# nreHieW/Eagle

Hardware: AMD Instinct MI355X
Metric: frames/sec end-to-end (detect+keypoint+homography) @1280x720 (higher is better)
Workload: dtype f32 (split: hi/lo binary16 pairs, 3 x fp16 MFMA per product, fp32 accumulate); detector (1.4 % of the FLOP): f32, exact v_mfma_f32_16x16x4_f32 chains

## Files before the change

eagle_amd/csrc/conv.hip:

```cpp
#include <algorithm>
#include <cmath>
#include <cstdlib>
#include <mutex>

#include "common.h"
#include "dmath.h"
#include "conv_internal.h"

namespace eagle {

static int f16_ps(int kc) { const int g = kc / 8; return kc * 2 + ((g % 2 == 0) ? 16 : 0); }
static int f16_ni(int ks, int kc) { return (ks * ks * (kc / 8) + 3) / 4; }

enum FormKind { GENERIC, WSTAT, ADIRECT };
enum StrideForm { S1, S2D, S2T };
enum WeightImage { W_F32, W_F16, W_F16_S2D, W_SPLIT, W_SPLIT_AD, W_SPLIT_S2D, W_SPLIT_M32 };
struct Form {
    int prec, variant, kind;
    int pw;
    int sform, rows, cols;
    int kc, nt, halo_bufs;
    int wimage;
    int grid_cap;
    ConvKernelGetter get;
};
static constexpr Form gen(int prec, int variant, int pw, int wimage, int kind = GENERIC) { return {prec, variant, kind, pw, S1, 0, 0, 0, 0, 0, wimage, 0, nullptr}; }
static constexpr Form ad(int prec, int variant, int sform, int rows, int cols, int nt, int halo_bufs, int wimage, ConvKernelGetter get, int grid_cap = 0)
{
    return {prec, variant, ADIRECT, 0, sform, rows, cols, prec == EAGLE_PREC_F16 ? 32 : 16, nt, halo_bufs, wimage, grid_cap, get};
}
static constexpr int F16 = EAGLE_PREC_F16, F32 = EAGLE_PREC_F32, F32S = EAGLE_PREC_F32S;
static constexpr Form g_forms[] = {
    gen(F32, 0, 4, W_F32), gen(F32, 3, 2, W_F32), gen(F32, 4, 1, W_F32),
    gen(F16, 0, 4, W_F16), gen(F16, 2, 4, W_F16), gen(F16, 3, 2, W_F16), gen(F16, 4, 1, W_F16), gen(F16, 6, 4, W_F16, WSTAT), gen(F16, 7, 2, W_F16, WSTAT),
    ad(F16, 8, S1, 4, 32, 12, 2, W_F16, conv_ad_kernel_s1_bn192), ad(F16, 9, S1, 8, 32, 6, 2, W_F16, conv_ad_kernel_s1_bn96),
    ad(F16, 10, S2D, 4, 32, 12, 2, W_F16_S2D, conv_ad_kernel_s2_bn192), ad(F16, 11, S2D, 8, 32, 6, 2, W_F16_S2D, conv_ad_kernel_s2_bn96),
    gen(F32S, 0, 4, W_SPLIT), gen(F32S, 3, 2, W_SPLIT), gen(F32S, 18, 6, W_SPLIT),
    ad(F32S, 8, S1, 4, 32, 12, 2, W_SPLIT_AD, conv_ad_split_kernel_bn192), ad(F32S, 9, S1, 8, 32, 6, 2, W_SPLIT_AD, conv_ad_split_kernel_bn96),
    ad(F32S, 10, S2D, 4, 32, 12, 2, W_SPLIT_S2D, conv_ad_split_kernel_s2_bn192), ad(F32S, 11, S2D, 8, 32, 6, 2, W_SPLIT_S2D, conv_ad_split_kernel_s2_bn96),
    ad(F32S, 12, S1, 8, 32, 3, 2, W_SPLIT_AD, conv_ad_split_kernel48), ad(F32S, 13, S1, 16, 32, 3, 1, W_SPLIT_AD, conv_ad_split_kernel48sb),
    ad(F32S, 19, S1, 16, 32, 3, 2, W_SPLIT_AD, conv_ad_split_kernel48ring, 256),
    ad(F32S, 14, S2T, 4, 32, 12, 1, W_SPLIT_AD, conv_ad_split_kernel_s2t_bn192), ad(F32S, 15, S2T, 4, 32, 6, 1, W_SPLIT_AD, conv_ad_split_kernel_s2t_bn96),
    ad(F32S, 21, S1, 4, 32, 12, 2, W_SPLIT_M32, conv_ad_split32_kernel_bn192), ad(F32S, 22, S1, 8, 32, 6, 2, W_SPLIT_M32, conv_ad_split32_kernel_bn96),
    ad(F32S, 23, S1, 2, 64, 12, 2, W_SPLIT_M32, conv_ad_split32_kernel_w64_bn192), ad(F32S, 24, S1, 4, 64, 6, 2, W_SPLIT_M32, conv_ad_split32_kernel_w64_bn96)};

static const Form* find_form(int precision, int variant)
{
    for (const Form& f : g_forms)
        if (f.prec == precision && f.variant == variant) return &f;
    return nullptr;
}
static const Form& form_of(int precision, const ConvConfig& c)
{
    const Form* f = find_form(precision, c.variant);
    if (!f) fail(EAGLE_E_NOKERNEL, "no conv kernel form: prec=%d variant=%d", precision, c.variant);
    return *f;
}
static int kind_of(int precision, const ConvConfig& c) { const Form* f = find_form(precision, c.variant); return f ? f->kind : -1; }

static size_t lds_bytes(int precision, const ConvConfig& c)
{
    const Form& f = form_of(precision, c);
    if (f.kind == ADIRECT) {
        int hpix, rec, strips;
        if (precision == EAGLE_PREC_F16) { hpix = f.sform == S2D ? (f.rows + 1) * 33 : (f.rows + 2) * 34; rec = 96; strips = 4 * 32 * 112; }
        else if (f.wimage == W_SPLIT_M32) { hpix = (f.rows + 2) * (f.cols + 2); rec = 80; strips = 4 * 32 * 128; }
        else { hpix = f.sform == S2T ? (2 * f.rows + 1) * 66 : (f.rows + 2) * 34; rec = 96; strips = 4 * 16 * 208; }
        const int slabs = ((hpix * rec + 1023) / 1024 + 3) / 4 * 4;
        return (size_t)f.halo_bufs * slabs * 1024 + strips;
    }
    const int th = 4 * f.pw / c.wx, tw = 16 * c.wx;
    const int hw = (tw - 1) * c.stride + c.ks, hh = (th - 1) * c.stride + c.ks;
    const int bn = c.nt * 16;
    if (precision == EAGLE_PREC_F16) {
        const size_t operands = (size_t)f16_ni(c.ks, c.kc) * 4 * bn * 16 + (size_t)hh * hw * f16_ps(c.kc);
        const size_t strips = (size_t)4 * f.pw * 16 * (bn * 2 + 16);
        return f.kind == WSTAT ? operands + strips + 16 : std::max(operands + 16, strips);
    }
    if (precision == EAGLE_PREC_F32S) {
        const size_t operands = (size_t)f16_ni(c.ks, c.kc) * 2 * 4 * bn * 16 + (size_t)hh * hw * f16_ps(2 * c.kc);
        const size_t strips = (size_t)4 * f.pw * 16 * (bn * 4 + 16);
        return std::max(operands + 16, strips);
    }
    return (size_t)c.ks * c.ks * (c.kc / 4) * 4 * bn * 4 + (size_t)hh * hw * (c.kc + 1) * 4;
}

size_t conv_lds_bytes(int precision, const ConvConfig& c) { return lds_bytes(precision, c); }
void conv_tile_shape(int precision, const ConvConfig& c, int* th, int* tw)
{
    const Form& f = form_of(precision, c);
    *th = f.kind == ADIRECT ? f.rows : 4 * f.pw / c.wx; *tw = f.kind == ADIRECT ? f.cols : 16 * c.wx;
}

int conv_tiles_per_frame(int precision, const ConvConfig& c, int ho, int wo)
{
    int th, tw;
    conv_tile_shape(precision, c, &th, &tw);
    return ((wo + tw - 1) / tw) * ((ho + th - 1) / th);
}

static const Inst* generic_inst(int precision, const ConvConfig& c)
{
    for (auto part : {conv_inst_part0, conv_inst_part1, conv_inst_part2, conv_inst_part3, conv_inst_split0, conv_inst_split1, conv_inst_split2}) {
        int n = 0;
        const Inst* t = part(&n);
        for (int k = 0; k < n; ++k)
            if (t[k].prec == precision && t[k].ks == c.ks && t[k].s == c.stride && t[k].kc == c.kc && t[k].nt == c.nt && t[k].variant == c.variant) return &t[k];
    }
    return nullptr;
}
bool conv_supported(int precision, const ConvConfig& c)
{
    const Form* f = find_form(precision, c.variant);
    if (f && f->kind == ADIRECT) return c.ks == 3 && c.stride == (f->sform == S1 ? 1 : 2) && c.kc == f->kc && c.nt == f->nt;
    return f && generic_inst(precision, c);
}

struct Tuned { int ks, s, cin, cout, wo, kc, nt, wx, variant; };
static const Tuned g_tuned[] = {
#include "conv_tuned.inc"
    {0, 0, 0, 0, 0, 0, 0, 0, 0}};
static const Tuned g_tuned_f32[] = {
#include "conv_tuned_f32.inc"
    {0, 0, 0, 0, 0, 0, 0, 0, 0}};
static const Tuned g_tuned_split[] = {
#include "conv_tuned_split.inc"
    {0, 0, 0, 0, 0, 0, 0, 0, 0}};
static bool tuned_match(const Tuned& t, const ConvConfig& c, int wo, ConvConfig* q)
{
    if (t.ks != c.ks || t.s != c.stride || t.cin != c.cin || t.cout != c.cout_pad || t.wo != wo) return false;
    *q = c; q->kc = t.kc; q->nt = t.nt; q->wx = t.wx; q->variant = t.variant;
    return true;
}

static bool env_force(const char* name, int* a, int* b, int* c) { const char* f = getenv(name); return f && sscanf(f, "%d,%d,%d", a, b, c) == 3; }
static bool env_off(const char* name) { const char* e = getenv(name); return e && atoi(e) == 0; }

static const int g_nts[] = {6, 4, 3, 2, 1};
static ConvConfig with_ad(ConvConfig c, int kc, int v192, int v96)
{
    c.kc = kc;
    if (c.cout_pad % 192 == 0) { c.nt = 12; c.variant = v192; } else { c.nt = 6; c.variant = v96; }
    return c;
}

static ConvConfig choose_f32(ConvConfig c, int wo)
{
    ConvConfig q = c; q.kc = (c.cin < 16) ? 4 : 16;
    if (env_force("EAGLE_F32_FORCE", &q.nt, &q.wx, &q.variant) && (q.wx == 1 || q.wx == 2) && q.nt >= 1 && c.cout_pad % (16 * q.nt) == 0 &&
        conv_supported(EAGLE_PREC_F32, q) && lds_bytes(EAGLE_PREC_F32, q) <= 160 * 1024)
        return q;
    for (const Tuned& t : g_tuned_f32)
        if (tuned_match(t, c, wo, &q) && conv_supported(EAGLE_PREC_F32, q)) return q;
    c.nt = 1;
    for (int nt : g_nts)
        if (c.cout_pad % (16 * nt) == 0) { c.nt = nt; break; }
    c.kc = (c.cin < 16) ? 4 : 16;
    if (c.stride == 2 && c.ks == 3) {
        q = c; q.variant = 3;
        if (conv_supported(EAGLE_PREC_F32, q)) return q;
    }
    return c;
}

static ConvConfig choose_split(ConvConfig c, int wo, bool plain_epilogue)
{
    const int prec = EAGLE_PREC_F32S, cin = c.cin, cout = c.cout_pad;
    ConvConfig q = c;
    if (env_force("EAGLE_CONV_FORCE", &q.kc, &q.nt, &q.variant) && cin % q.kc == 0 && cout % (16 * q.nt) == 0 && conv_supported(prec, q)) {
        if (form_of(prec, q).pw == 6) q.wx = 3;
        if (lds_bytes(prec, q) <= 160 * 1024) return q;
    }
    if (plain_epilogue && c.ks == 3 && c.stride == 2 && cin % 48 == 0 && cout % 96 == 0) return with_ad(c, 16, 14, 15);
    if (!env_off("EAGLE_CONV_M32") && plain_epilogue && c.ks == 3 && c.stride == 1 && cin % 16 == 0 && cout % 96 == 0) return with_ad(c, 16, 21, wo > 32 ? 24 : 22);
    for (const Tuned& t : g_tuned_split)
        if (tuned_match(t, c, wo, &q)) {
            const Form* f = find_form(prec, q.variant);
            if (kind_of(prec, q) == ADIRECT && !(plain_epilogue && cin % (f->sform == S2D ? 16 : 48) == 0)) continue;
            if (conv_supported(prec, q) && lds_bytes(prec, q) <= 160 * 1024) return q;
        }
    if (plain_epilogue && c.ks == 3 && c.stride == 1 && cin % 48 == 0 && cout % 96 == 0) return with_ad(c, 16, 8, 9);
    static const int skcs[] = {32, 16, 8};
    long best = -1;
    c.nt = 1; c.kc = 8; c.variant = 0;
    for (int variant : {0, 3})
        for (int nt : g_nts) {
            if (cout % (16 * nt)) continue;
            for (int kc : skcs) {
                if (cin % kc) continue;
                ConvConfig t = c; t.nt = nt; t.kc = kc; t.variant = variant;
                if (!conv_supported(prec, t)) continue;
                if (lds_bytes(prec, t) > 80 * 1024) continue;
                const int pw = form_of(prec, t).pw;
                if (nt * pw > 12) continue;
                const long score = (long)nt * pw * 1000 + kc * 10 + (variant == 0 ? 1 : 0);
                if (score > best) { best = score; c.nt = nt; c.kc = kc; c.variant = variant; }
            }
        }
    return c;
}

static ConvConfig choose_f16(ConvConfig c, int wo, bool plain_epilogue, bool plain_one)
{
    const int prec = EAGLE_PREC_F16, cin = c.cin, cout = c.cout_pad;
    ConvConfig q = c;
    if (env_force("EAGLE_CONV_FORCE", &q.kc, &q.nt, &q.variant) && cin % q.kc == 0 && cout % (16 * q.nt) == 0 && conv_supported(prec, q) &&
        lds_bytes(prec, q) <= 160 * 1024 && (kind_of(prec, q) == WSTAT ? plain_one : kind_of(prec, q) == ADIRECT ? plain_epilogue : true))
        return q;
    if (plain_epilogue && c.ks == 3 && c.stride == 1 && cin % 32 == 0 && cout % 96 == 0) return with_ad(c, 32, 8, 9);
    if (plain_epilogue && c.ks == 3 && c.stride == 2 && cin % 8 == 0 && cin >= 32 && cout % 96 == 0) return with_ad(c, 32, 10, 11);
    for (const Tuned& t : g_tuned)
        if (tuned_match(t, c, wo, &q)) {
            if (kind_of(prec, q) == WSTAT && !plain_one) continue;
            if (conv_supported(prec, q) && lds_bytes(prec, q) <= 160 * 1024) return q;
        }
    static const int kcs[] = {64, 48, 32, 16, 8};
    long best = -1;
    c.nt = 1; c.kc = 8;
    for (int nt : g_nts) {
        if (cout % (16 * nt)) continue;
        for (int kc : kcs) {
            if (cin % kc) continue;
            ConvConfig t = c; t.nt = nt; t.kc = kc;
            if (!conv_supported(prec, t)) continue;
            if (lds_bytes(prec, t) > 80 * 1024) continue;
            const long score = (long)kc * nt * 1000 + kc;
            if (score > best) { best = score; c.nt = nt; c.kc = kc; }
        }
    }
    return c;
}

ConvConfig conv_choose(int precision, int ks, int stride, int cin_pad, int cout_pad, int wo, bool plain_epilogue, bool second_residual)
{
    ConvConfig c;
    c.ks = ks; c.stride = stride; c.cin = cin_pad; c.cout_pad = cout_pad;
    c.wx = (wo > 16) ? 2 : 1;
    if (precision == EAGLE_PREC_F32) return choose_f32(c, wo);
    if (precision == EAGLE_PREC_F32S) return choose_split(c, wo, plain_epilogue);
    return choose_f16(c, wo, plain_epilogue, plain_epilogue && !second_residual);
}

size_t conv_weight_elems(int precision, const ConvConfig& c)
{
    const int bn = c.nt * 16, nblk = c.cout_pad / bn, nch = c.cin / c.kc;
    switch (form_of(precision, c).wimage) {
    case W_F16_S2D: return (size_t)nblk * (4 * c.cin / 32) * 16 * bn * 8;
    case W_F16: return (size_t)nblk * nch * f16_ni(c.ks, c.kc) * 4 * bn * 8;
    case W_SPLIT_S2D: return (size_t)nblk * (4 * c.cin / 16) * 6 * 4 * bn * 8;
    case W_SPLIT_M32: return (size_t)nblk * (c.cin / 16) * 18 * (bn / 32) * 512;
    case W_SPLIT_AD: return (size_t)nblk * (c.cin / 16) * 14 * 4 * bn * 8;
    case W_SPLIT: return (size_t)nblk * nch * f16_ni(c.ks, c.kc) * 2 * 4 * bn * 8;
    default: return (size_t)nblk * nch * c.ks * c.ks * (c.kc / 4) * 4 * bn;
    }
}

void conv_tile_weights(int precision, const ConvConfig& c, const float* w, int cin_real, int cout_real, void* dst, float* descale)
{
    const int bn = c.nt * 16, nblk = c.cout_pad / bn, nch = c.cin / c.kc, taps = c.ks * c.ks, wimage = form_of(precision, c).wimage;
    auto W = [&](int tap, int ci, int co) -> float {
        return (ci < cin_real && co < cout_real) ? w[((size_t)tap * cin_real + ci) * cout_real + co] : 0.0f;
    };
    if (descale) *descale = 1.0f;
    if (precision == EAGLE_PREC_F32S) {
        float amax = 0.f;
        for (size_t k = 0; k < (size_t)taps * cin_real * cout_real; ++k) amax = std::max(amax, std::fabs(w[k]));
        int e = 0;
        if (amax > 0.f) (void)std::frexp(amax, &e);
        const int sw = 15 - e;
        const float scale = std::ldexp(1.0f, sw);
        if (descale) *descale = std::ldexp(1.0f, -(sw + 4));
        _Float16* d = (_Float16*)dst;
        if (wimage == W_SPLIT_S2D) {
            const int per_phase = c.cin / 16;
            for (int b = 0; b < nblk; ++b)
                for (int ch = 0; ch < 4 * per_phase; ++ch)
                    for (int k = 0; k < 6; ++k)
                        for (int qq = 0; qq < 4; ++qq)
                            for (int nn = 0; nn < bn; ++nn)
                                for (int j = 0; j < 8; ++j) {
                                    const int ph = ch / per_phase, c0 = (ch - ph * per_phase) * 16, ry = ph >> 1, rx = ph & 1;
                                    const int tp = k < 4 ? k : 2 * (k - 4) + (qq >> 1), tyy = tp >> 1, txx = tp & 1;
                                    const int ky = tyy == 0 ? (ry == 1 ? 0 : -1) : (ry == 0 ? 1 : 2), kx = txx == 0 ? (rx == 1 ? 0 : -1) : (rx == 0 ? 1 : 2);
                                    float v = 0.f;
                                    if (ky >= 0 && kx >= 0) v = W(ky * 3 + kx, c0 + (qq & 1) * 8 + j, b * bn + nn) * scale;
                                    const _Float16 hi = (_Float16)v;
                                    *d++ = k < 4 ? hi : (_Float16)(v - (float)hi);
                                }
            return;
        }
        if (wimage == W_SPLIT_M32) {
            for (int b = 0; b < nblk; ++b)
                for (int ch = 0; ch < c.cin / 16; ++ch)
                    for (int tap = 0; tap < 9; ++tap)
                        for (int part = 0; part < 2; ++part)
                            for (int mb = 0; mb < bn / 32; ++mb)
                                for (int l = 0; l < 64; ++l)
                                    for (int j = 0; j < 8; ++j) {
                                        const float v = W(tap, ch * 16 + (l >> 5) * 8 + j, b * bn + mb * 32 + (l & 31)) * scale;
                                        const _Float16 hi = (_Float16)v;
                                        *d++ = part == 0 ? hi : (_Float16)(v - (float)hi);
                                    }
            return;
        }
        if (wimage == W_SPLIT_AD) {
            for (int b = 0; b < nblk; ++b)
                for (int ch = 0; ch < c.cin / 16; ++ch)
                    for (int k = 0; k < 14; ++k)
                        for (int qq = 0; qq < 4; ++qq)
                            for (int nn = 0; nn < bn; ++nn)
                                for (int j = 0; j < 8; ++j) {
                                    const int tap = k < 9 ? k : 2 * (k - 9) + (qq >> 1);
                                    float v = 0.f;
                                    if (tap < 9) v = W(tap, ch * 16 + (qq & 1) * 8 + j, b * bn + nn) * scale;
                                    const _Float16 hi = (_Float16)v;
                                    *d++ = k < 9 ? hi : (_Float16)(v - (float)hi);
                                }
            return;
        }
        const int G = c.kc / 8, NGR = taps * G, NI = f16_ni(c.ks, c.kc);
        for (int b = 0; b < nblk; ++b)
            for (int ch = 0; ch < nch; ++ch)
                for (int i = 0; i < NI; ++i)
                    for (int part = 0; part < 2; ++part)
                        for (int qq = 0; qq < 4; ++qq)
                            for (int nn = 0; nn < bn; ++nn)
                                for (int j = 0; j < 8; ++j) {
                                    const int g = 4 * i + qq;
                                    float v = 0.f;
                                    if (g < NGR) { const int tap = g / G, cg = g % G; v = W(tap, ch * c.kc + cg * 8 + j, b * bn + nn) * scale; }
                                    const _Float16 hi = (_Float16)v;
                                    *d++ = part == 0 ? hi : (_Float16)(v - (float)hi);
                                }
        return;
    }
    if (wimage == W_F16_S2D) {
        _Float16* d = (_Float16*)dst;
        const int nch2 = 4 * c.cin / 32;
        for (int b = 0; b < nblk; ++b)
            for (int ch = 0; ch < nch2; ++ch)
                for (int g = 0; g < 16; ++g)
                    for (int nn = 0; nn < bn; ++nn)
                        for (int j = 0; j < 8; ++j) {
                            const int tp = g / 4, cg = g % 4, tyy = tp >> 1, txx = tp & 1;
                            const int sc = ch * 32 + cg * 8 + j, ph = sc / c.cin, ci = sc - ph * c.cin, ry = ph >> 1, rx = ph & 1;
                            const int ky = tyy == 0 ? (ry == 1 ? 0 : -1) : (ry == 0 ? 1 : 2), kx = txx == 0 ? (rx == 1 ? 0 : -1) : (rx == 0 ? 1 : 2);
                            *d++ = (_Float16)((ky < 0 || kx < 0) ? 0.f : W(ky * 3 + kx, ci, b * bn + nn));
                        }
        return;
    }
    if (precision == EAGLE_PREC_F16) {
        const int G = c.kc / 8, NGR = taps * G, NI = f16_ni(c.ks, c.kc);
        _Float16* d = (_Float16*)dst;
        for (int b = 0; b < nblk; ++b)
            for (int ch = 0; ch < nch; ++ch)
                for (int g = 0; g < NI * 4; ++g)
                    for (int nn = 0; nn < bn; ++nn)
                        for (int j = 0; j < 8; ++j) {
                            float v = 0.f;
                            if (g < NGR) {
                                const int tap = g / G, cg = g % G;
                                v = W(tap, ch * c.kc + cg * 8 + j, b * bn + nn);
                            }
                            *d++ = (_Float16)v;
                        }
    } else {
        const int CSTEPS = c.kc / 4;
        float* d = (float*)dst;
        for (int b = 0; b < nblk; ++b)
            for (int ch = 0; ch < nch; ++ch)
                for (int tap = 0; tap < taps; ++tap)
                    for (int cs = 0; cs < CSTEPS; ++cs)
                        for (int qq = 0; qq < 4; ++qq)
                            for (int nn = 0; nn < bn; ++nn) *d++ = W(tap, ch * c.kc + cs * 4 + qq, b * bn + nn);
    }
}

static std::mutex g_page_mutex;
static const void* conv_zero_page()
{
    static void* z[64] = {};
    int dev = 0;
    HIP_CHECK(hipGetDevice(&dev));
    std::lock_guard<std::mutex> g(g_page_mutex);
    if (!z[dev]) { HIP_CHECK(hipMalloc(&z[dev], 256)); HIP_CHECK(hipMemset(z[dev], 0, 256)); }
    return z[dev];
}
static void* conv_trash_page()
{
    static void* z[64] = {};
    int dev = 0;
    HIP_CHECK(hipGetDevice(&dev));
    std::lock_guard<std::mutex> g(g_page_mutex);
    if (!z[dev]) HIP_CHECK(hipMalloc(&z[dev], 8192));
    return z[dev];
}

void conv_launch(int precision, const ConvLaunch& L, hipStream_t s)
{
    const ConvConfig& c = L.cfg;
    if (!conv_supported(precision, c)) fail(EAGLE_E_NOKERNEL, "no conv kernel instance: prec=%d ks=%d s=%d kc=%d nt=%d", precision, c.ks, c.stride, c.kc, c.nt);
    const Form& f = form_of(precision, c);
    ConvArgs a;
    a.x = L.x.p; a.xcs = L.x.cs; a.xoff = L.x.off; a.N = L.x.n; a.H = L.x.h; a.W = L.x.w;
    a.w = L.w; a.bias = L.bias;
    a.y = L.y.p; a.ycs = L.y.cs; a.yoff = L.y.off; a.Ho = L.y.h; a.Wo = L.y.w;
    a.r1 = L.r1.p; a.r1cs = L.r1.cs; a.r1off = L.r1.off;
    a.r2 = L.r2.p; a.r2cs = L.r2.cs; a.r2off = L.r2.off;
    a.descale = L.descale;
    if (precision == EAGLE_PREC_F32S) {
        if (L.x.f32 != 2 || (L.r1.p && L.r1.f32 != 2) || (L.r2.p && L.r2.f32 != 2) || L.y.f32 != (L.out_f32 ? 1 : 2))
            fail(EAGLE_E_INVALID, "split conv: operand tensor formats do not match the family");
        a.xcs *= 2; a.xoff *= 2; a.r1cs *= 2; a.r1off *= 2; a.r2cs *= 2; a.r2off *= 2;
        if (!L.out_f32) { a.ycs *= 2; a.yoff *= 2; }
    }
    if (!a.r1 && a.r2) { a.r1 = a.r2; a.r1cs = a.r2cs; a.r1off = a.r2off; a.r2 = nullptr; }
    a.pre_act = L.pre_act; a.post_act = L.post_act; a.out_f32 = L.out_f32 || precision == EAGLE_PREC_F32;
    a.wx = c.wx;
    a.nchunks = c.cin / c.kc;
    a.zeros = conv_zero_page(); a.trash = conv_trash_page(); a.xcd = 0; a.gy = 1; a.stack = 0;
    a.am = L.am_slot ? *L.am_slot : nullptr; a.am_cs = c.cout_pad;
    a.sat = (L.sat_slot && precision == EAGLE_PREC_F32S) ? *L.sat_slot : nullptr;
    if (f.kind == ADIRECT) {
        if (a.out_f32 || a.pre_act != 0 || a.post_act > 1 || L.am_slot || (precision == EAGLE_PREC_F32S && c.cin % (f.wimage == W_SPLIT_AD ? 48 : 16)))
            fail(EAGLE_E_NOKERNEL, "A-direct conv needs 2-byte / split output, pre_act none, post_act in {none, ReLU} and, in the split family, Cin = 16 k (48 k for variants 8, 9 and 12 - 15)");
        if (f.sform == S2D) a.nchunks = 4 * c.cin / c.kc;
        a.tiles_x = (a.Wo + f.cols - 1) / f.cols; a.tiles_y = (a.Ho + f.rows - 1) / f.rows;
        a.gy = c.cout_pad / (c.nt * 16);
        const size_t lim = (size_t)1 << 31;
        if ((size_t)a.N * a.H * a.W * a.xcs * 2 >= lim || (size_t)a.N * a.Ho * a.Wo * std::max(std::max(a.ycs, a.r1 ? a.r1cs : 0), a.r2 ? a.r2cs : 0) * 2 >= lim)
            fail(EAGLE_E_INVALID, "fp16 conv: a tensor of %d frames reaches 2 GiB; use a smaller device batch", a.N);
        const int nres = (a.r1 ? 1 : 0) + (a.r2 ? 1 : 0);
        const int items = a.tiles_x * a.tiles_y * a.N * a.gy;
        const bool deep = items <= 256;
        for (bool d : {false, true}) ensure_max_dynamic_lds((const void*)f.get(nres, d), 160 * 1024);
        hipLaunchKernelGGL(f.get(nres, deep), dim3(f.grid_cap ? std::min(items, f.grid_cap) : items), dim3(256), lds_bytes(precision, c), s, a);
        HIP_CHECK(hipGetLastError());
        return;
    }
    const int th = 4 * f.pw / c.wx, tw = 16 * c.wx;
    a.tiles_x = (a.Wo + tw - 1) / tw; a.tiles_y = (a.Ho + th - 1) / th;
    if (precision == EAGLE_PREC_F32) {
        if (!env_off("EAGLE_F32_STACK") && c.stride == 1 && a.N > 1 && a.Ho == a.H) { a.stack = 1; a.tiles_y = (a.N * (a.Ho + 1) + th - 1) / th; }
        if ((size_t)a.N * a.H * a.W * a.xcs * 4 >= ((size_t)1 << 31)) fail(EAGLE_E_INVALID, "fp32 conv: the input tensor of %d frames reaches 2 GiB; use a smaller device batch", a.N);
    }
    const bool ws = f.kind == WSTAT;
    if (a.am && (!prec_is_f16_kernels(precision) || ws))
        fail(EAGLE_E_NOKERNEL, "fused heat-map maxima need the generic fp16 kernel");
    if (prec_is_f16_kernels(precision)) {
        const size_t lim = (size_t)1 << 31;
        const size_t cs_out = std::max(std::max(a.out_f32 ? 2 * a.ycs : a.ycs, a.r1 ? a.r1cs : 0), a.r2 ? a.r2cs : 0);
        if ((size_t)a.N * a.H * a.W * a.xcs * 2 >= lim || (size_t)a.N * a.Ho * a.Wo * cs_out * 2 >= lim)
            fail(EAGLE_E_INVALID, "fp16 conv: a tensor of %d frames reaches 2 GiB; use a smaller device batch", a.N);
    }
    const ConvKernel fn = generic_inst(precision, c)->fn;
    const size_t lds = lds_bytes(precision, c);
    ensure_max_dynamic_lds((const void*)fn, 160 * 1024);
    const int gy = c.cout_pad / (c.nt * 16);
    int gx = a.stack ? a.tiles_x * a.tiles_y : a.tiles_x * a.tiles_y * a.N;
    if (ws) {
        if (c.kc != c.cin || a.out_f32 || a.r2 || a.pre_act != 0 || a.post_act > 1 || (size_t)a.N * a.H * a.W * a.xcs * 2 >= (1ull << 31) || (size_t)a.N * a.Ho * a.Wo * std::max(a.ycs, a.r1 ? a.r1cs : 0) * 2 >= (1ull << 31))
            fail(EAGLE_E_NOKERNEL, "weight-stationary conv needs kc == cin, fp16 output, at most one residual, pre_act none, post_act in {none, ReLU} and tensors below 2 GiB (kc=%d cin=%d)", c.kc, c.cin);
        const int per_cu = (int)std::max<size_t>(1, std::min<size_t>(2, (160 * 1024) / lds));
        const int unit = 8 * gy;
        gx = std::max(unit, std::min((gx * gy + unit - 1) / unit * unit, 256 * per_cu / unit * unit));
    }
    a.gy = gy;
    a.xcd = (prec_is_f16_kernels(precision) && !ws && (c.ks == 3 || (c.ks == 1 && gy > 1))) ? 1 : 0;
    dim3 grid(gx, gy);
    if (a.xcd) grid = dim3(gx * gy, 1);
    if (ws) grid = dim3(gx, 1);
    hipLaunchKernelGGL(fn, grid, dim3(256), lds, s, a);
    HIP_CHECK(hipGetLastError());
}

}
```

eagle_amd/csrc/conv_ad_split32.hip:

```cpp
#include <algorithm>
#include <cstdlib>
#include <type_traits>

#include "common.h"
#include "dmath.h"
#include "conv_internal.h"

namespace eagle {

#include "conv_kernels.inc"
#include "conv_ad_split32.inc"

ConvKernel conv_ad_split32_kernel_bn192(int n_res, bool deep)
{
    static const ConvKernel fn[2][3] = {
        {conv_split_ad32_kernel<2, 2, 0>, conv_split_ad32_kernel<2, 2, 1>, conv_split_ad32_kernel<2, 2, 2>},
        {conv_split_ad32_kernel<2, 2, 0, 6>, conv_split_ad32_kernel<2, 2, 1, 6>, conv_split_ad32_kernel<2, 2, 2, 6>}};
    return fn[deep ? 1 : 0][res_slot(n_res)];
}

ConvKernel conv_ad_split32_kernel_bn96(int n_res, bool deep)
{
    static const ConvKernel fn[2][3] = {
        {conv_split_ad32_kernel<1, 4, 0>, conv_split_ad32_kernel<1, 4, 1>, conv_split_ad32_kernel<1, 4, 2>},
        {conv_split_ad32_kernel<1, 4, 0, 6>, conv_split_ad32_kernel<1, 4, 1, 6>, conv_split_ad32_kernel<1, 4, 2, 6>}};
    return fn[deep ? 1 : 0][res_slot(n_res)];
}

ConvKernel conv_ad_split32_kernel_w64_bn192(int n_res, bool deep)
{
    static const ConvKernel fn[2][3] = {
        {conv_split_ad32_kernel<2, 2, 0, 3, 2>, conv_split_ad32_kernel<2, 2, 1, 3, 2>, conv_split_ad32_kernel<2, 2, 2, 3, 2>},
        {conv_split_ad32_kernel<2, 2, 0, 6, 2>, conv_split_ad32_kernel<2, 2, 1, 6, 2>, conv_split_ad32_kernel<2, 2, 2, 6, 2>}};
    return fn[deep ? 1 : 0][res_slot(n_res)];
}

ConvKernel conv_ad_split32_kernel_w64_bn96(int n_res, bool deep)
{
    static const ConvKernel fn[2][3] = {
        {conv_split_ad32_kernel<1, 4, 0, 3, 2>, conv_split_ad32_kernel<1, 4, 1, 3, 2>, conv_split_ad32_kernel<1, 4, 2, 3, 2>},
        {conv_split_ad32_kernel<1, 4, 0, 6, 2>, conv_split_ad32_kernel<1, 4, 1, 6, 2>, conv_split_ad32_kernel<1, 4, 2, 6, 2>}};
    return fn[deep ? 1 : 0][res_slot(n_res)];
}

}
```

eagle_amd/csrc/conv_ad_split32.inc:

```
#ifndef EAGLE_CONV_AD_SPLIT32_INC
#define EAGLE_CONV_AD_SPLIT32_INC
#ifndef EAGLE_ABL_M32
#define EAGLE_ABL_M32 0
#endif
#ifndef EAGLE_M32_RES_NT
#define EAGLE_M32_RES_NT 1
#endif
#ifndef EAGLE_M32_SAUX
#define EAGLE_M32_SAUX (EAGLE_STORE_NT * 2 + EAGLE_M32_RES_NT * 4)
#endif
using f32x16 = __attribute__((ext_vector_type(16))) float;
#if EAGLE_ABL_M32 == 1 || EAGLE_ABL_M32 == 6
__device__ __forceinline__ f32x16 abl_m32_xor(const half8& a_, const half8& b_, f32x16 c_)
{
    const u32x4 ua = __builtin_bit_cast(u32x4, a_), ub = __builtin_bit_cast(u32x4, b_);
    c_[0] = __builtin_bit_cast(float, __builtin_bit_cast(unsigned, c_[0]) ^ ua[0] ^ ub[3]);
    return c_;
}
#define EAGLE_MFMA_M32(A_, B_, C_) abl_m32_xor(A_, B_, C_)
#else
#define EAGLE_MFMA_M32(A_, B_, C_) __builtin_amdgcn_mfma_f32_32x32x16_f16(A_, B_, C_, 0, 0, 0)
#endif
__device__ __forceinline__ void split_store4x(char* dhi, char* dlo, float v0, float v1, float v2, float v3)
{
    const float s0 = __builtin_amdgcn_fmed3f(v0 * SPLIT_SX, -65504.0f, 65504.0f), s1 = __builtin_amdgcn_fmed3f(v1 * SPLIT_SX, -65504.0f, 65504.0f),
                s2 = __builtin_amdgcn_fmed3f(v2 * SPLIT_SX, -65504.0f, 65504.0f), s3 = __builtin_amdgcn_fmed3f(v3 * SPLIT_SX, -65504.0f, 65504.0f);
    const half4 hi = {(_Float16)s0, (_Float16)s1, (_Float16)s2, (_Float16)s3};
    const half4 lo = {(_Float16)(s0 - (float)hi[0]), (_Float16)(s1 - (float)hi[1]), (_Float16)(s2 - (float)hi[2]), (_Float16)(s3 - (float)hi[3])};
    *(half4*)dhi = hi; *(half4*)dlo = lo;
}
template <int CQ, int PG, int RES, int RING = 3, int NRH = 1>
__global__ __launch_bounds__(256, 2) void conv_split_ad32_kernel(ConvArgs a)
{
    static_assert(CQ * PG == 4, "four waves per workgroup");
    static_assert(NRH == 1 || NRH == 2, "the wave's two pixel blocks: one above the other (1) or side by side (2)");
    static_assert(18 % RING == 0 && RING >= 3, "the weight ring holds a divisor of the 18 steps of a chunk");
    using rsrc_t = __amdgpu_buffer_rsrc_t;
    constexpr unsigned OOB = 0x80000000u;
    constexpr int MB = 3, NR = 2, NRV = NR / NRH, NW = 4, BN = CQ * 96, TH = NRV * PG, TW = 32 * NRH;
    constexpr int KSTEP = (BN / 32) * 1024;
    constexpr int PS = 80, SPC = 18, AHEAD = RING - 1;
    constexpr int HW_ = TW + 2, HPIX = (TH + 2) * HW_;
    constexpr int HSLABS = ((HPIX * PS + 1023) / 1024 + NW - 1) / NW * NW, HB = HSLABS * 1024, HK = HSLABS / NW;
    constexpr int RS = 32 * 4, STRIP = 32 * RS;
    extern __shared__ __attribute__((aligned(16))) char smem[];
    char* const Hb = smem;
    char* const strip = smem + 2 * HB + (threadIdx.x >> 6) * STRIP;
    const int tid = threadIdx.x, lane = tid & 63, wave = __builtin_amdgcn_readfirstlane(tid >> 6);
    const int cq = wave % CQ, pg = wave / CQ, kh = lane >> 5, lx = lane & 31;
    const int gy = a.gy, nitems = a.tiles_x * a.tiles_y * a.N * gy, nwg = gridDim.x;
    int item0, item_end;
    {
        const int b = blockIdx.x, xcd = b & 7, k = b >> 3;
        const int wgs_here = (nwg + 7 - xcd) >> 3;
        const int qn = nitems >> 3, rn = nitems & 7;
        const int x0 = xcd < rn ? xcd * (qn + 1) : rn * (qn + 1) + (xcd - rn) * qn;
        const int xc = qn + (xcd < rn ? 1 : 0);
        item0 = x0 + (int)((long)xc * k / wgs_here);
        item_end = x0 + (int)((long)xc * (k + 1) / wgs_here);
    }
    if (item0 >= item_end) return;
    const int nloc = item_end - item0, nch = a.nchunks, GC = nloc * nch;
    const rsrc_t xrs = __builtin_amdgcn_make_buffer_rsrc((void*)a.x, 0, 0x7FFFFFFF, 0x00020000);
    const rsrc_t wrs = __builtin_amdgcn_make_buffer_rsrc((void*)a.w, 0, 0x7FFFFFFF, 0x00020000);
    const rsrc_t rrs = __builtin_amdgcn_make_buffer_rsrc((void*)a.r1, 0, 0x7FFFFFFF, 0x00020000);
    const rsrc_t rrs2 = __builtin_amdgcn_make_buffer_rsrc((void*)a.r2, 0, 0x7FFFFFFF, 0x00020000);
    const rsrc_t yrs = __builtin_amdgcn_make_buffer_rsrc((void*)a.y, 0, 0x7FFFFFFF, 0x00020000);
    constexpr bool RECOMP = HK > 6;
    const int e0 = wave * 64 + lane;
    int hpk[RECOMP ? 1 : HK];
    if constexpr (!RECOMP) {
#pragma unroll
        for (int k = 0; k < HK; ++k) {
            const int e = e0 + NW * 64 * k;
            const int pix = e / 5, slot = e - pix * 5;
            const int hy = pix / HW_, hx = pix - hy * HW_;
            hpk[k] = (pix < HPIX && slot < 4) ? (hy | (hx << 8) | (((slot & 1) * 2 + (slot >> 1)) << 16)) : -1;
        }
    }
    const int bbase = ((pg * NRV) * HW_ + lx) * PS + kh * 16;
    const unsigned wlane = (unsigned)((cq * MB * 64 + lane) * 16);

    auto decode = [&](int item, int& n, int& ty, int& tx, int& nb) {
        int t = item / gy; nb = item - t * gy;
        tx = t % a.tiles_x; t /= a.tiles_x;
        ty = t % a.tiles_y; n = t / a.tiles_y;
    };
    int h_g = 0, h_ch = 0, h_item = item0;
    int h_iy0, h_ix0, h_gb;
    auto halo_origin = [&](int item) {
        int n, ty, tx, nb; decode(item, n, ty, tx, nb);
        h_iy0 = ty * TH - 1; h_ix0 = tx * TW - 1;
        h_gb = (((n * a.H + h_iy0) * a.W + h_ix0) * a.xcs + a.xoff) * 2;
    };
    halo_origin(h_item);
    auto issue_h_slab = [&](int k) {
        char* dst = Hb + (h_g & 1) * HB;
        const unsigned so = (EAGLE_ABL_M32 == 8) ? 0u : (unsigned)(h_ch * 32) * 2u;
        int hy, hx, unit; bool live;
        if constexpr (RECOMP) {
            int e = e0 + NW * 64 * k;
            asm volatile("" : "+v"(e));
            const int pix = (int)(((unsigned)e * 52429u) >> 18), slot = e - pix * 5;
            hy = HW_ == 34 ? (int)(((unsigned)pix * 1928u) >> 16) : (int)(((unsigned)pix * 993u) >> 16); hx = pix - hy * HW_;
            unit = (slot & 1) * 2 + (slot >> 1);
            live = pix < HPIX && slot < 4;
        } else {
            hy = hpk[k] & 0xFF; hx = (hpk[k] >> 8) & 0xFF; unit = (hpk[k] >> 16) & 7; live = hpk[k] >= 0;
        }
        const int iy = h_iy0 + hy, ix = h_ix0 + hx;
        const unsigned off = !(live && (unsigned)iy < (unsigned)a.H && (unsigned)ix < (unsigned)a.W) ? OOB
                             : (unsigned)(h_gb + ((hy * a.W + hx) * a.xcs + unit * 8) * 2);
        __builtin_amdgcn_raw_ptr_buffer_load_lds(xrs, (__attribute__((address_space(3))) void*)(dst + (wave + NW * k) * 1024), 16,
                                                 ((EAGLE_ABL_M32 == 3 || EAGLE_ABL_M32 == 6 || EAGLE_ABL_M32 == 7) && h_g > 0) ? OOB : off, so, 0, 0);
    };
    auto advance_h = [&]() {
        if (h_g + 1 >= GC) return;
        ++h_g;
        if (++h_ch == nch) { h_ch = 0; ++h_item; halo_origin(h_item); }
    };
    auto issue_h = [&]() {
#pragma unroll
        for (int k = 0; k < HK; ++k) issue_h_slab(k);
        advance_h();
    };
    issue_h();
    int gc = 0;
    for (int item = item0; item < item_end; ++item) {
        int n, ty, tx, nb; decode(item, n, ty, tx, nb);
        const int oy0 = ty * TH, ox0 = tx * TW;
        f32x16 acc[MB][NR];
#pragma unroll
        for (int i = 0; i < MB; ++i)
#pragma unroll
            for (int p = 0; p < NR; ++p)
#pragma unroll
                for (int r = 0; r < 16; ++r) acc[i][p][r] = 0.f;
        u32x4 A[RING][MB];
        unsigned wsrc = (unsigned)(nb * nch * SPC) * (unsigned)KSTEP;
        const unsigned wend = wsrc + (unsigned)(nch * SPC) * (unsigned)KSTEP;
        bool abl_a_done = false;
        auto load_a = [&](int slot) {
            const unsigned so = wsrc < wend ? wsrc : wend - KSTEP;
#pragma unroll
            for (int mb = 0; mb < MB; ++mb)
                if (!((EAGLE_ABL_M32 == 2 || EAGLE_ABL_M32 == 6 || EAGLE_ABL_M32 == 7) && abl_a_done)) A[slot][mb] = __builtin_amdgcn_raw_buffer_load_b128(wrs, wlane + mb * 1024, so, 0);
            wsrc += KSTEP;
        };
#pragma unroll
        for (int s = 0; s < AHEAD; ++s) load_a(s);
        abl_a_done = true;
        for (int ch = 0; ch < nch; ++ch, ++gc) {
            if constexpr (AHEAD * MB == 6) asm volatile("s_waitcnt vmcnt(6)" ::: "memory");
            else asm volatile("s_waitcnt vmcnt(15)" ::: "memory");
            static_assert(AHEAD * MB == 6 || AHEAD * MB == 15, "vmcnt literal");
            __builtin_amdgcn_s_barrier();
            issue_h();
            const char* hb = Hb + (gc & 1) * HB + bbase;
            half8 Bh[2][NR], Bl[2][NR];
            auto read_b = [&](int slot, int tap) {
                const int ky = tap / 3, kx = tap - ky * 3;
#pragma unroll
                for (int p = 0; p < NR; ++p) {
                    Bh[slot][p] = *(const half8*)(hb + ((p / NRH + ky) * HW_ + (p % NRH) * 32 + kx) * PS);
                    Bl[slot][p] = *(const half8*)(hb + ((p / NRH + ky) * HW_ + (p % NRH) * 32 + kx) * PS + 32);
                }
            };
            read_b(0, 0);
#pragma unroll
            for (int t = 0; t < 9; ++t) {
                const int bs = (EAGLE_ABL_M32 == 4 || EAGLE_ABL_M32 == 6) ? 0 : (t & 1);
                load_a((2 * t + AHEAD) % RING);
                if (t + 1 < 9 && !(EAGLE_ABL_M32 == 4 || EAGLE_ABL_M32 == 6)) read_b((t + 1) & 1, t + 1);
#pragma unroll
                for (int p = 0; p < NR; ++p)
#pragma unroll
                    for (int mb = 0; mb < MB; ++mb) acc[mb][p] = EAGLE_MFMA_M32((half8)A[(2 * t) % RING][mb], Bh[bs][p], acc[mb][p]);
#pragma unroll
                for (int p = 0; p < NR; ++p)
#pragma unroll
                    for (int mb = 0; mb < MB; ++mb) acc[mb][p] = EAGLE_MFMA_M32((half8)A[(2 * t) % RING][mb], Bl[bs][p], acc[mb][p]);
                __builtin_amdgcn_sched_barrier(0);
                load_a((2 * t + 1 + AHEAD) % RING);
#pragma unroll
                for (int p = 0; p < NR; ++p)
#pragma unroll
                    for (int mb = 0; mb < MB; ++mb) acc[mb][p] = EAGLE_MFMA_M32((half8)A[(2 * t + 1) % RING][mb], Bh[bs][p], acc[mb][p]);
                __builtin_amdgcn_sched_barrier(0);
            }
        }
        const int co0 = nb * BN + cq * 96;
        __builtin_amdgcn_sched_barrier(0);
        const float ds = a.descale;
        int pstrip[4], ppx[4];
#pragma unroll
        for (int i = 0; i < 4; ++i) {
            const int e = i * 64 + lane, px = e >> 3, u = e & 7;
            pstrip[i] = px * RS + ((u ^ (px & 7)) * 16);
            ppx[i] = px | (u << 8);
        }
        auto piece_off = [&](int pass, int i, int cs, int off) -> unsigned {
            const int row = pass / MB, mb = pass - row * MB;
            const int oy = oy0 + pg * NRV + row / NRH, ox2 = ox0 + (row % NRH) * 32 + (ppx[i] & 0xFF), u = ppx[i] >> 8;
            return (oy < a.Ho && ox2 < a.Wo) ? (unsigned)((((n * a.Ho + oy) * a.Wo + ox2) * cs + off + (co0 + mb * 32) * 2 + u * 8) * 2) : OOB;
        };
        float vmax = 0.0f;
        constexpr int NPASS = NR * MB, PB = (RES == 2 && NRH == 2) ? 2 : (RES == 2 || (RES == 1 && NRH == 2)) ? 3 : 6;
        u32x4 rres[RES >= 1 ? PB : 1][4], rres2[RES >= 2 ? PB : 1][4];
        char* const sp = strip + lx * RS + kh * 8;
        const int sw = (lx & 7) * 16;
        auto run_hi = [&](int j) -> char* { return sp + ((j * 32) ^ sw); };
        auto run_lo = [&](int j) -> char* { return sp + ((j * 32 + 16) ^ sw); };
#pragma unroll
        for (int pb0 = 0; pb0 < NPASS; pb0 += PB) {
            if (RES >= 1) {
#pragma unroll
                for (int h2 = 0; h2 < PB; ++h2)
#pragma unroll
                    for (int i = 0; i < 4; ++i) rres[h2][i] = __builtin_amdgcn_raw_buffer_load_b128(rrs, piece_off(pb0 + h2, i, a.r1cs, a.r1off), 0, (EAGLE_M32_SAUX & 4) ? 2 : 0);
            }
            if (RES >= 2) {
#pragma unroll
                for (int h2 = 0; h2 < PB; ++h2)
#pragma unroll
                    for (int i = 0; i < 4; ++i) rres2[h2][i] = __builtin_amdgcn_raw_buffer_load_b128(rrs2, piece_off(pb0 + h2, i, a.r2cs, a.r2off), 0, (EAGLE_M32_SAUX & 4) ? 2 : 0);
            }
#pragma unroll
            for (int h2 = 0; h2 < PB; ++h2) {
                const int pass = pb0 + h2, row = pass / MB, mb = pass - row * MB;
                if (RES >= 1) {
#pragma unroll
                    for (int i = 0; i < 4; ++i) *(u32x4*)(strip + pstrip[i]) = rres[h2][i];
                }
                float v[4][4];
#pragma unroll
                for (int j = 0; j < 4; ++j) {
                    const float4 bv = *(const float4*)(a.bias + co0 + mb * 32 + j * 8 + kh * 4);
                    v[j][0] = acc[mb][row][j * 4 + 0] * ds + bv.x; v[j][1] = acc[mb][row][j * 4 + 1] * ds + bv.y;
                    v[j][2] = acc[mb][row][j * 4 + 2] * ds + bv.z; v[j][3] = acc[mb][row][j * 4 + 3] * ds + bv.w;
                    if (RES >= 1) {
                        const half4 rh = *(const half4*)run_hi(j), rl = *(const half4*)run_lo(j);
#pragma unroll
                        for (int r = 0; r < 4; ++r) v[j][r] = ((float)rh[r] + (float)rl[r]) * SPLIT_RX + v[j][r];
                    }
                }
                if (RES >= 2) {
#pragma unroll
                    for (int i = 0; i < 4; ++i) *(u32x4*)(strip + pstrip[i]) = rres2[h2][i];
#pragma unroll
                    for (int j = 0; j < 4; ++j) {
                        const half4 rh = *(const half4*)run_hi(j), rl = *(const half4*)run_lo(j);
#pragma unroll
                        for (int r = 0; r < 4; ++r) v[j][r] = v[j][r] + ((float)rh[r] + (float)rl[r]) * SPLIT_RX;
                    }
                }
#pragma unroll
                for (int j = 0; j < 4; ++j) {
                    if (a.post_act == 1) {
#pragma unroll
                        for (int r = 0; r < 4; ++r) v[j][r] = v[j][r] > 0.f ? v[j][r] : 0.f;
                    }
                    split_store4x(run_hi(j), run_lo(j), v[j][0], v[j][1], v[j][2], v[j][3]);
                    vmax = split_absmax4(vmax, v[j][0], v[j][1], v[j][2], v[j][3]);
                }
#pragma unroll
                for (int i = 0; i < 4; ++i)
                    __builtin_amdgcn_raw_buffer_store_b128(*(const u32x4*)(strip + pstrip[i]), yrs, (EAGLE_ABL_M32 >= 5 && EAGLE_ABL_M32 <= 7) ? OOB : piece_off(pass, i, a.ycs, a.yoff), 0, EAGLE_M32_SAUX & 3);
            }
        }
        split_report(a.sat, n, vmax);
    }
}

#endif
```

eagle_amd/csrc/conv_internal.h:

```cpp
#pragma once
#include "common.h"

namespace eagle {

using half8 = __attribute__((ext_vector_type(8))) _Float16;
using half4 = __attribute__((ext_vector_type(4))) _Float16;
using f32x4 = __attribute__((ext_vector_type(4))) float;
using u32x4 = __attribute__((ext_vector_type(4))) unsigned int;
using u32x2 = __attribute__((ext_vector_type(2))) unsigned int;

struct ConvArgs {
    const void* x; int xcs, xoff; int N, H, W;
    const void* w; const float* bias;
    void* y; int ycs, yoff; int Ho, Wo;
    const void* r1; int r1cs, r1off;
    const void* r2; int r2cs, r2off;
    int pre_act, post_act, out_f32;
    int wx, tiles_x, tiles_y, nchunks;
    int gy;
    int stack;
    int xcd;
    ArgmaxPart* am;
    int am_cs;
    float descale;
    const void* zeros;
    void* trash;
    unsigned* sat;
};

struct BneckArgs {
    const void* x; int xcs, xoff; int N, H, W, nch1;
    const void *w1, *w2, *w3; const float *b1, *b2, *b3; float ds1, ds2, ds3;
    const void* r; int rcs, roff;
    void* y; int ycs, yoff;
    int tiles_x, tiles_y;
    unsigned* sat;
    unsigned long long* dbg;
};

typedef void (*ConvKernel)(ConvArgs);
struct Inst { int prec, ks, s, kc, nt, variant; ConvKernel fn; };
const Inst* conv_inst_part0(int* n); const Inst* conv_inst_part1(int* n); const Inst* conv_inst_part2(int* n); const Inst* conv_inst_part3(int* n);
const Inst* conv_inst_split0(int* n); const Inst* conv_inst_split1(int* n); const Inst* conv_inst_split2(int* n);
inline int res_slot(int n_res) { return n_res < 0 ? 0 : n_res > 2 ? 2 : n_res; }
typedef ConvKernel (*ConvKernelGetter)(int n_res, bool deep);
ConvKernel conv_ad_kernel_s1_bn192(int n_res, bool deep);
ConvKernel conv_ad_kernel_s1_bn96(int n_res, bool deep);
ConvKernel conv_ad_kernel_s2_bn192(int n_res, bool deep);
ConvKernel conv_ad_kernel_s2_bn96(int n_res, bool deep);
ConvKernel conv_ad_split_kernel_bn192(int n_res, bool deep);
ConvKernel conv_ad_split_kernel_bn96(int n_res, bool deep);
ConvKernel conv_ad_split_kernel_s2_bn192(int n_res, bool deep);
ConvKernel conv_ad_split_kernel_s2_bn96(int n_res, bool deep);
ConvKernel conv_ad_split_kernel_s2t_bn192(int n_res, bool deep);
ConvKernel conv_ad_split_kernel_s2t_bn96(int n_res, bool deep);
ConvKernel conv_ad_split_kernel48(int n_res, bool deep);
ConvKernel conv_ad_split_kernel48sb(int n_res, bool deep);
ConvKernel conv_ad_split_kernel48ring(int n_res, bool deep);
ConvKernel conv_ad_split32_kernel_bn192(int n_res, bool deep);
ConvKernel conv_ad_split32_kernel_bn96(int n_res, bool deep);
ConvKernel conv_ad_split32_kernel_w64_bn192(int n_res, bool deep);
ConvKernel conv_ad_split32_kernel_w64_bn96(int n_res, bool deep);

}
```

Baseline: 827.6.

## Add linear pixel tiling variant of split32 conv for 30-column maps

Adds a new A-direct split-fp16 conv form that tiles the output as runs of 128 flattened pixels, rather than 4x32 rectangular tiles. The aim is to avoid wasting lanes on 30-wide feature maps, where a 32-wide tile leaves columns idle. Halo loads cover the rows spanned by each linear run, and per-lane B-operand addresses are precomputed from the row/column of each flattened pixel. In exchange, the halo holds extra rows, address arithmetic is more irregular, and the form is restricted to maps exactly 30 wide with matching input size.

New measurement: 837.2, median of 6. 1.2% higher.

```diff
diff --git a/eagle_amd/csrc/conv.hip b/eagle_amd/csrc/conv.hip
--- a/eagle_amd/csrc/conv.hip
+++ b/eagle_amd/csrc/conv.hip
@@ -13,7 +13,7 @@
 static int f16_ni(int ks, int kc) { return (ks * ks * (kc / 8) + 3) / 4; }
 
 enum FormKind { GENERIC, WSTAT, ADIRECT };
-enum StrideForm { S1, S2D, S2T };
+enum StrideForm { S1, S2D, S2T, S1L };
 enum WeightImage { W_F32, W_F16, W_F16_S2D, W_SPLIT, W_SPLIT_AD, W_SPLIT_S2D, W_SPLIT_M32 };
 struct Form {
     int prec, variant, kind;
@@ -42,7 +42,9 @@
     ad(F32S, 19, S1, 16, 32, 3, 2, W_SPLIT_AD, conv_ad_split_kernel48ring, 256),
     ad(F32S, 14, S2T, 4, 32, 12, 1, W_SPLIT_AD, conv_ad_split_kernel_s2t_bn192), ad(F32S, 15, S2T, 4, 32, 6, 1, W_SPLIT_AD, conv_ad_split_kernel_s2t_bn96),
     ad(F32S, 21, S1, 4, 32, 12, 2, W_SPLIT_M32, conv_ad_split32_kernel_bn192), ad(F32S, 22, S1, 8, 32, 6, 2, W_SPLIT_M32, conv_ad_split32_kernel_bn96),
-    ad(F32S, 23, S1, 2, 64, 12, 2, W_SPLIT_M32, conv_ad_split32_kernel_w64_bn192), ad(F32S, 24, S1, 4, 64, 6, 2, W_SPLIT_M32, conv_ad_split32_kernel_w64_bn96)};
+    ad(F32S, 23, S1, 2, 64, 12, 2, W_SPLIT_M32, conv_ad_split32_kernel_w64_bn192), ad(F32S, 24, S1, 4, 64, 6, 2, W_SPLIT_M32, conv_ad_split32_kernel_w64_bn96),
+    ad(F32S, 27, S1L, 6, 30, 12, 2, W_SPLIT_M32, conv_ad_split32_kernel_lin30)};
+static constexpr int LIN_PIXELS = 128;
 
 static const Form* find_form(int precision, int variant)
 {
@@ -96,6 +98,7 @@
 {
     int th, tw;
     conv_tile_shape(precision, c, &th, &tw);
+    if (form_of(precision, c).sform == S1L) return (ho * wo + LIN_PIXELS - 1) / LIN_PIXELS;
     return ((wo + tw - 1) / tw) * ((ho + th - 1) / th);
 }
 
@@ -112,7 +115,7 @@
 bool conv_supported(int precision, const ConvConfig& c)
 {
     const Form* f = find_form(precision, c.variant);
-    if (f && f->kind == ADIRECT) return c.ks == 3 && c.stride == (f->sform == S1 ? 1 : 2) && c.kc == f->kc && c.nt == f->nt;
+    if (f && f->kind == ADIRECT) return c.ks == 3 && c.stride == (f->sform == S1 || f->sform == S1L ? 1 : 2) && c.kc == f->kc && c.nt == f->nt;
     return f && generic_inst(precision, c);
 }
 
@@ -167,12 +170,17 @@
 {
     const int prec = EAGLE_PREC_F32S, cin = c.cin, cout = c.cout_pad;
     ConvConfig q = c;
-    if (env_force("EAGLE_CONV_FORCE", &q.kc, &q.nt, &q.variant) && cin % q.kc == 0 && cout % (16 * q.nt) == 0 && conv_supported(prec, q)) {
+    if (env_force("EAGLE_CONV_FORCE", &q.kc, &q.nt, &q.variant) && cin % q.kc == 0 && cout % (16 * q.nt) == 0 && conv_supported(prec, q) &&
+        (form_of(prec, q).sform != S1L || (plain_epilogue && wo == form_of(prec, q).cols))) {
         if (form_of(prec, q).pw == 6) q.wx = 3;
         if (lds_bytes(prec, q) <= 160 * 1024) return q;
     }
     if (plain_epilogue && c.ks == 3 && c.stride == 2 && cin % 48 == 0 && cout % 96 == 0) return with_ad(c, 16, 14, 15);
-    if (!env_off("EAGLE_CONV_M32") && plain_epilogue && c.ks == 3 && c.stride == 1 && cin % 16 == 0 && cout % 96 == 0) return with_ad(c, 16, 21, wo > 32 ? 24 : 22);
+    if (!env_off("EAGLE_CONV_M32") && plain_epilogue && c.ks == 3 && c.stride == 1 && cin % 16 == 0 && cout % 96 == 0) {
+        q = with_ad(c, 16, 21, wo > 32 ? 24 : 22);
+        if (q.variant == 21 && wo == 30) q.variant = 27;
+        return q;
+    }
     for (const Tuned& t : g_tuned_split)
         if (tuned_match(t, c, wo, &q)) {
             const Form* f = find_form(prec, q.variant);
@@ -426,6 +434,10 @@
             fail(EAGLE_E_NOKERNEL, "A-direct conv needs 2-byte / split output, pre_act none, post_act in {none, ReLU} and, in the split family, Cin = 16 k (48 k for variants 8, 9 and 12 - 15)");
         if (f.sform == S2D) a.nchunks = 4 * c.cin / c.kc;
         a.tiles_x = (a.Wo + f.cols - 1) / f.cols; a.tiles_y = (a.Ho + f.rows - 1) / f.rows;
+        if (f.sform == S1L) {
+            if (a.Wo != f.cols || a.W != a.Wo || a.H != a.Ho) fail(EAGLE_E_NOKERNEL, "linear A-direct conv (variant %d) needs a map %d columns wide, got %d x %d", c.variant, f.cols, a.Ho, a.Wo);
+            a.tiles_x = (a.Ho * a.Wo + LIN_PIXELS - 1) / LIN_PIXELS; a.tiles_y = 1;
+        }
         a.gy = c.cout_pad / (c.nt * 16);
         const size_t lim = (size_t)1 << 31;
         if ((size_t)a.N * a.H * a.W * a.xcs * 2 >= lim || (size_t)a.N * a.Ho * a.Wo * std::max(std::max(a.ycs, a.r1 ? a.r1cs : 0), a.r2 ? a.r2cs : 0) * 2 >= lim)
diff --git a/eagle_amd/csrc/conv_ad_split32.hip b/eagle_amd/csrc/conv_ad_split32.hip
--- a/eagle_amd/csrc/conv_ad_split32.hip
+++ b/eagle_amd/csrc/conv_ad_split32.hip
@@ -43,4 +43,12 @@
     return fn[deep ? 1 : 0][res_slot(n_res)];
 }
 
+ConvKernel conv_ad_split32_kernel_lin30(int n_res, bool deep)
+{
+    static const ConvKernel fn[2][3] = {
+        {conv_split_ad32_kernel<2, 2, 0, 3, 1, 30>, conv_split_ad32_kernel<2, 2, 1, 3, 1, 30>, conv_split_ad32_kernel<2, 2, 2, 3, 1, 30>},
+        {conv_split_ad32_kernel<2, 2, 0, 6, 1, 30>, conv_split_ad32_kernel<2, 2, 1, 6, 1, 30>, conv_split_ad32_kernel<2, 2, 2, 6, 1, 30>}};
+    return fn[deep ? 1 : 0][res_slot(n_res)];
 }
+
+}
diff --git a/eagle_amd/csrc/conv_ad_split32.inc b/eagle_amd/csrc/conv_ad_split32.inc
--- a/eagle_amd/csrc/conv_ad_split32.inc
+++ b/eagle_amd/csrc/conv_ad_split32.inc
@@ -29,10 +29,12 @@
     const half4 lo = {(_Float16)(s0 - (float)hi[0]), (_Float16)(s1 - (float)hi[1]), (_Float16)(s2 - (float)hi[2]), (_Float16)(s3 - (float)hi[3])};
     *(half4*)dhi = hi; *(half4*)dlo = lo;
 }
-template <int CQ, int PG, int RES, int RING = 3, int NRH = 1>
+template <int CQ, int PG, int RES, int RING = 3, int NRH = 1, int MAPW = 0>
 __global__ __launch_bounds__(256, 2) void conv_split_ad32_kernel(ConvArgs a)
 {
     static_assert(CQ * PG == 4, "four waves per workgroup");
+    constexpr bool LIN = MAPW != 0;
+    static_assert(!LIN || (CQ == 2 && PG == 2 && NRH == 1 && MAPW == 30), "linear tiling: the BN = 192 form on the 30-column map");
     static_assert(NRH == 1 || NRH == 2, "the wave's two pixel blocks: one above the other (1) or side by side (2)");
     static_assert(18 % RING == 0 && RING >= 3, "the weight ring holds a divisor of the 18 steps of a chunk");
     using rsrc_t = __amdgpu_buffer_rsrc_t;
@@ -40,7 +42,8 @@
     constexpr int MB = 3, NR = 2, NRV = NR / NRH, NW = 4, BN = CQ * 96, TH = NRV * PG, TW = 32 * NRH;
     constexpr int KSTEP = (BN / 32) * 1024;
     constexpr int PS = 80, SPC = 18, AHEAD = RING - 1;
-    constexpr int HW_ = TW + 2, HPIX = (TH + 2) * HW_;
+    constexpr int LROWS = LIN ? (128 - 2) / (LIN ? MAPW : 1) + 2 : 0;
+    constexpr int HW_ = LIN ? MAPW + 2 : TW + 2, HPIX = (LIN ? LROWS + 2 : TH + 2) * HW_;
     constexpr int HSLABS = ((HPIX * PS + 1023) / 1024 + NW - 1) / NW * NW, HB = HSLABS * 1024, HK = HSLABS / NW;
     constexpr int RS = 32 * 4, STRIP = 32 * RS;
     extern __shared__ __attribute__((aligned(16))) char smem[];
@@ -90,7 +93,8 @@
     int h_iy0, h_ix0, h_gb;
     auto halo_origin = [&](int item) {
         int n, ty, tx, nb; decode(item, n, ty, tx, nb);
-        h_iy0 = ty * TH - 1; h_ix0 = tx * TW - 1;
+        if constexpr (LIN) { h_iy0 = (tx * 128) / MAPW - 1; h_ix0 = -1; }
+        else { h_iy0 = ty * TH - 1; h_ix0 = tx * TW - 1; }
         h_gb = (((n * a.H + h_iy0) * a.W + h_ix0) * a.xcs + a.xoff) * 2;
     };
     halo_origin(h_item);
@@ -129,6 +133,16 @@
     for (int item = item0; item < item_end; ++item) {
         int n, ty, tx, nb; decode(item, n, ty, tx, nb);
         const int oy0 = ty * TH, ox0 = tx * TW;
+        const int L0 = tx * 128, npix = a.H * a.W;
+        int bbl[LIN ? NR : 1];
+        if constexpr (LIN) {
+            const int yf = L0 / MAPW;
+#pragma unroll
+            for (int p = 0; p < NR; ++p) {
+                const int L = min(L0 + (pg * NR + p) * 32 + lx, npix - 1), y = L / MAPW, x = L - y * MAPW;
+                bbl[p] = ((y - yf) * HW_ + x) * PS + kh * 16;
+            }
+        }
         f32x16 acc[MB][NR];
 #pragma unroll
         for (int i = 0; i < MB; ++i)
@@ -157,13 +171,23 @@
             __builtin_amdgcn_s_barrier();
             issue_h();
             const char* hb = Hb + (gc & 1) * HB + bbase;
+            const char* hbl[LIN ? NR : 1];
+            if constexpr (LIN) {
+#pragma unroll
+                for (int p = 0; p < NR; ++p) hbl[p] = Hb + (gc & 1) * HB + bbl[p];
+            }
             half8 Bh[2][NR], Bl[2][NR];
             auto read_b = [&](int slot, int tap) {
                 const int ky = tap / 3, kx = tap - ky * 3;
 #pragma unroll
                 for (int p = 0; p < NR; ++p) {
-                    Bh[slot][p] = *(const half8*)(hb + ((p / NRH + ky) * HW_ + (p % NRH) * 32 + kx) * PS);
-                    Bl[slot][p] = *(const half8*)(hb + ((p / NRH + ky) * HW_ + (p % NRH) * 32 + kx) * PS + 32);
+                    if constexpr (LIN) {
+                        Bh[slot][p] = *(const half8*)(hbl[p] + (ky * HW_ + kx) * PS);
+                        Bl[slot][p] = *(const half8*)(hbl[p] + (ky * HW_ + kx) * PS + 32);
+                    } else {
+                        Bh[slot][p] = *(const half8*)(hb + ((p / NRH + ky) * HW_ + (p % NRH) * 32 + kx) * PS);
+                        Bl[slot][p] = *(const half8*)(hb + ((p / NRH + ky) * HW_ + (p % NRH) * 32 + kx) * PS + 32);
+                    }
                 }
             };
             read_b(0, 0);
@@ -201,6 +225,10 @@
         }
         auto piece_off = [&](int pass, int i, int cs, int off) -> unsigned {
             const int row = pass / MB, mb = pass - row * MB;
+            if constexpr (LIN) {
+                const int L = L0 + (pg * NR + row) * 32 + (ppx[i] & 0xFF), u = ppx[i] >> 8;
+                return L < npix ? (unsigned)(((n * npix + L) * cs + off + (co0 + mb * 32) * 2 + u * 8) * 2) : OOB;
+            }
             const int oy = oy0 + pg * NRV + row / NRH, ox2 = ox0 + (row % NRH) * 32 + (ppx[i] & 0xFF), u = ppx[i] >> 8;
             return (oy < a.Ho && ox2 < a.Wo) ? (unsigned)((((n * a.Ho + oy) * a.Wo + ox2) * cs + off + (co0 + mb * 32) * 2 + u * 8) * 2) : OOB;
         };
diff --git a/eagle_amd/csrc/conv_internal.h b/eagle_amd/csrc/conv_internal.h
--- a/eagle_amd/csrc/conv_internal.h
+++ b/eagle_amd/csrc/conv_internal.h
@@ -61,5 +61,6 @@
 ConvKernel conv_ad_split32_kernel_bn96(int n_res, bool deep);
 ConvKernel conv_ad_split32_kernel_w64_bn192(int n_res, bool deep);
 ConvKernel conv_ad_split32_kernel_w64_bn96(int n_res, bool deep);
+ConvKernel conv_ad_split32_kernel_lin30(int n_res, bool deep);
 
 }
```
